# pkuyzy/ESC-GNN

Measured on AMD Instinct MI355X. Metric: graphs/sec + edges-aggregated/sec, NestedGIN_eff h=3 bs=128 @1/2/4/8 GPU, higher is better.
Workload: dtype f32; 1 GPU; count_cycle-shaped random regular graphs (n in 10/15/20/30), target=triangles, NestedGIN_eff h=3 layers=4 hidden=256, bs=128 per GPU (configs[1]); global_batch=128, parallelism=dp1 graph-sharded, rccl_ranks=1, ranks=1

## Files before the change

### esc-gnn_amd/_native.py

```python
import ctypes
import os
from ctypes import c_double, c_float, c_int, c_int64, c_void_p, POINTER

_HERE = os.path.dirname(os.path.abspath(__file__))
LIB_PATH = os.path.join(_HERE, "libescgnn_hip.so")
ABI_VERSION = 4

P, I64, I32, F32 = c_void_p, c_int64, c_int, c_float

class CollateArgs(ctypes.Structure):
    _fields_ = ([(n, c_int64) for n in ("B", "x_dim", "y_dim", "n_cols")] +
                [(n, c_void_p) for n in (
                    "graph_ids", "offsets", "node_ptr", "edge_ptr", "nnz_ptr", "y_ptr", "x_all", "y_all",
                    "esrc_all", "edst_all", "pos_enc_all", "pos_index_all", "pos_batch_all",
                    "in_ptr_all", "in_edge_all", "out_ptr_all", "out_edge_all", "row_ptr_all", "c_perm_all",
                    "c_rank_all", "col_ptr", "col_prefix",
                    "x", "y", "edge_index", "batch", "pos_enc", "pos_index", "pos_batch",
                    "in_ptr", "in_edge", "in_src", "out_ptr", "out_edge", "out_dst",
                    "row_ptr", "bag_idx", "bag_val", "col_row", "col_val", "col_col", "edge_attr_all", "edge_attr")] +
                [("ea_words", c_int64), ("x_long", c_void_p), ("graph_ptr", c_void_p)])

class BnFuse(ctypes.Structure):
    _fields_ = [("eps", c_float), ("momentum", c_float)] + [(n, c_void_p) for n in (
        "mean", "invstd", "running_mean", "running_var", "gamma", "beta", "scale", "shift")]
# ... 57 lines not shown
    "esc_plan_csr_scratch": [I64, I64],
    "esc_plan_csr": [P, I64, I64, P, P, P, P, P],
    "esc_embed_plan_scratch": [I64, I64, I64],
    "esc_embed_plan": [P, I64, I64, P, P, P, P, P, P, P, P, P, P],
    "esc_tune_set": [I32, I32],
    "esc_debug_gemm_occupancy": [I32],
    "esc_linear_bwd_input": [P, I64, P, I64, I64, I64, I64, P, I64, I32, P],
    "esc_linear_bwd_weight_scratch": [I64, I64, I64],
    "esc_linear_bwd_weight": [P, I64, P, I64, P, P, I64, I64, I64, P, I64, P, P, P],
    "esc_linear_bwd_both": [P, I64, P, I64, P, P, P, I64, I64, I64, I64, P, I64, I32, P, I64, P, P, P],
    "esc_linear_bwd_both_deferred": [P, I64, P, I64, P, P, P, I64, I64, I64, I64, P, I64, I32, P, I64, P, P, P, P],
    "esc_slab_reduce_jobs": [P, I32, P],
    "esc_linear_bwd_both_bn_ok": [P, I64, POINTER(BnBwdFused), P, I64, P, I64, I64, I64, I64, P, I64, P, POINTER(BnBwdNext)],
    "esc_linear_bwd_bn_block_rows": [I64, I64, I64],
    "esc_linear_bwd_set_wgrad_stream": [P],
    "esc_linear_bwd_both_bn": [P, I64, POINTER(BnBwdFused), P, I64, P, P, P, I64, I64, I64, I64, P, I64, I32, P, I64, P, P, P,
                               POINTER(BnBwdNext), P],
    "esc_bn_bwd_coef": [P, I64, P, I64, P, I64, I64, I64, P, P, P, P, I32, P, P, P, P, P],
    "esc_bn_bwd_coef_from_partials": [P, I64, I64, I64, P, P, P, P],
    "esc_bn_scratch": [I64],
    "esc_bn_stats": [P, I64, I64, I64, F32, F32, P, P, P, P, P, P, P, P, P, P],
    "esc_bn_stats_from_partials": [P, I64, I64, F32, F32, P, P, P, P, P, P, P, P, P],
    "esc_bn_apply": [P, I64, I64, I64, P, P, P, P, I32, P, I64, P],
    "esc_bn_bwd": [P, I64, P, I64, P, I64, I64, I64, P, P, P, P, I32, P, I64, P, P, P, P],
    "esc_bn_bwd_sums": [P, I64, P, I64, P, I64, I64, I64, P, P, P, P, I32, P, P, P, P, P],
    "esc_bn_bwd_apply": [P, I64, P, I64, P, I64, I64, I64, P, P, P, P, I32, P, P, I64, P],
    "esc_affine_act": [P, I64, I64, I64, P, P, I32, P, I64, P],
    "esc_bn_eval_coef": [P, P, P, P, F32, I64, P, P, P],
    "esc_engine_set_side_stream": [I32],
    "esc_engine_set_materialise_edge_act": [I32],
# ... 130 lines not shown
```

### esc-gnn_amd/csrc/engine.hip

```cpp
#include "common.h"

#include <cstring>
#include <map>
#include <vector>
#include <cstdlib>

namespace esc {

struct Arena {
  float* base;
  int64_t off;
  float* take(int64_t n) {
    float* p = base ? base + off : nullptr;
    off += (n + 63) & ~63LL;
    return p;
  }
};

struct BnWs { float *mean, *invstd, *scale, *shift, *nglob, *coef; };
struct MlpWs { float *Y0, *Y1; BnWs b0, b1; float* A1 = nullptr; };

struct Layout {
  int64_t N, E, Z, H, L, C0, W;
  float *Zb, *Yz; BnWs zb0, zb1;
// ... 165 lines not shown

struct SideStream {
  hipStream_t stream = nullptr;
  hipEvent_t fork_f = nullptr, join_f = nullptr, fork_b = nullptr, join_b = nullptr;
  bool ok = false;
};
static int g_materialise_edge_act = 1;
static int g_use_side_stream = 0;

struct EdgeStream {
  hipStream_t stream = nullptr;
  hipEvent_t z_ready = nullptr, joined = nullptr, lin1_fork = nullptr, lin1_rest = nullptr, tail_dz = nullptr, e_ready[ESC_MAX_LAYERS] = {}, de_ready[ESC_MAX_LAYERS] = {},
             agg_done[ESC_MAX_LAYERS] = {};
  bool ok = false;
};
static int g_split_last_lin = getenv("ESC_SPLIT_LAST_LIN") ? atoi(getenv("ESC_SPLIT_LAST_LIN")) : 1;
static int g_edge_priority_low = 1;
static int g_use_edge_stream = 1;
static int current_device() {
  int dev = 0;
  (void)hipGetDevice(&dev);
  return dev;
}
static EdgeStream& edge_stream() {
  static thread_local std::map<int, EdgeStream> per_device;
  static thread_local EdgeStream off;
  if (!g_use_edge_stream) return off;
  EdgeStream& es = per_device[current_device()];
  if (!es.ok && es.stream == nullptr) {
    int least = 0, greatest = 0;
// ... 562 lines not shown
    (void)hipEventRecord(ss.join_b, ss.stream);
  }
  Ctx ce = es.ok ? edge_ctx(c, es.stream) : c;
  std::vector<esc_reduce_job> edge_jobs;
  edge_jobs.reserve(ESC_MAX_REDUCE_JOBS);
  if (es.ok && c.jobs) ce.jobs = &edge_jobs;
  std::vector<esc_sum_job> eps_jobs;
  int64_t agg_slots = 0;
  for (int l = (int)L - 1; l >= 0; --l) {
    const esc_conv_t& cv = m->conv[l];
    const int64_t C = l == 0 ? y.C0 : H;
    const float* hin = l == 0 ? b->x : y.cat + (int64_t)l * H;
    const int64_t ld_h = l == 0 ? y.C0 : W;
    Ctx cl = c;
    if (c.wgrad) { cl.y.dT1 = y.dT1_l[l]; cl.y.dT2 = y.dT2_l[l]; }
    ESC_TRY(mlp_backward(cl, cv.nn, y.conv[l], y.agg[l], C, N, y.cat + (int64_t)(l + 1) * H, W,
                         y.dcat + (int64_t)(l + 1) * H, W, y.dagg, C, fuse_node_act(c), l == (int)L - 1 ? last_slots : agg_slots));
    agg_slots = 0;
    float* dx = l == 0 ? nullptr : y.dcat + (int64_t)l * H;
    if (split_lin1 && l == (int)L - 1 &&
        hipStreamWaitEvent((hipStream_t)c.s, es.lin1_rest, 0) != hipSuccess) { set_error("esc_engine: stream event failed"); return ESC_ELAUNCH; }
    const bool stats_here = fuse_node_act(c) && l > 0 && (g_bn_fuse_bwd & 8) && esc_gine_aggregate_bwd_deps_slots(C) == 1 && C <= 2048 &&
                            mlp_backward_fused(c, m->conv[l - 1].nn, y.conv[l - 1], y.agg[l - 1], l - 1 == 0 ? y.C0 : H, N, y.cat + (int64_t)l * H, W,
                                               y.dcat + (int64_t)l * H, W, y.dagg, l - 1 == 0 ? y.C0 : H, true);
    if (stats_here) {
      ESC_TRY(esc_gine_aggregate_bwd_affine_stats(hin, ld_h, y.cat_scale + (int64_t)l * H, y.cat_shift + (int64_t)l * H, y.conv[l - 1].b1.mean,
                                                  y.conv[l - 1].b1.invstd, y.e[l], y.ld_e[l], y.dagg, C, b->out_ptr, b->out_edge, b->out_dst, cv.eps, N, C,
                                                  y.d_e[l], C, dx, W, 1, y.deps_part + (int64_t)l * 2 * N, y.bst_part, c.s));
      agg_slots = esc_gine_aggregate_bwd_stats_slots(N);
    } else if (fuse_node_act(c) && l > 0)
      ESC_TRY(esc_gine_aggregate_bwd_affine(hin, ld_h, y.cat_scale + (int64_t)l * H, y.cat_shift + (int64_t)l * H, y.e[l], y.ld_e[l], y.dagg, C,
                                            b->out_ptr, b->out_edge, b->out_dst, cv.eps, N, C, y.d_e[l], C, dx, W, 1,
                                            y.deps_part + (int64_t)l * 2 * N, c.s));
    else
      ESC_TRY(esc_gine_aggregate_bwd(hin, ld_h, y.e[l], y.ld_e[l], y.dagg, C, b->out_ptr, b->out_edge, b->out_dst, cv.eps, N, C,
                                     y.d_e[l], C, dx, W, 1, y.deps_part + (int64_t)l * 2 * N, c.s));
    eps_jobs.push_back(esc_sum_job{y.deps_part + (int64_t)l * 2 * N, N * esc_gine_aggregate_bwd_deps_slots(C), cv.deps});
    if (es.ok) ESC_TRY(chain(es.de_ready[l], (hipStream_t)c.s, es.stream));
    const float* zin = g_materialise_edge_act ? y.Zemb : y.Yz;
    const float* zsc = g_materialise_edge_act ? nullptr : y.zb1.scale;
    const float* zsh = g_materialise_edge_act ? nullptr : y.zb1.shift;
    if (l == 0 && es.ok && c.jobs && g_split_last_lin) {
      {
        const LdsFloorGuard cap(true);
        ESC_TRY(esc_linear_bwd_input(y.d_e[l], C, cv.lin.w, H, E, C, H, y.dZemb, H, l == (int)L - 1 ? 0 : 1, es.stream));
      }
      float* slabs = *c.slab_cursor;
      *c.slab_cursor += (esc_linear_bwd_weight_scratch(E, C, H) + 63) & ~63LL;
      c.jobs->emplace_back();
      ESC_TRY(esc_linear_bwd_both_deferred(y.d_e[l], C, zin, H, zsc, zsh, cv.lin.w, H, E, C, H, nullptr, 0, 0, cv.lin.dw, H, cv.lin.db,
                                           slabs, &c.jobs->back(), c.s));
    } else {
      ESC_TRY(linear_backward(ce, y.d_e[l], C, zin, H, zsc, zsh, cv.lin, E, y.dZemb, H, l == (int)L - 1 ? 0 : 1));
// ... 952 lines not shown
```

### esc-gnn_amd/csrc/linear_mfma.hip

```cpp
#include "common.h"
#include <array>
#include <cstdlib>
#include <map>
#include "gemm_dma.h"
#include "linear_small.h"
#include <type_traits>

namespace esc {

typedef float f32x16 __attribute__((ext_vector_type(16)));

constexpr int KPAD = 4;

template <int ROWS, int BK, int NTHR = 256>
struct KContigTile {
  static constexpr int LD = BK + KPAD;
  static constexpr int FLOATS = ROWS * LD;
  static constexpr int QPR = BK / 4;
  static constexpr int PER_THREAD = ROWS * QPR / NTHR;
  static_assert(ROWS * QPR % NTHR == 0 && NTHR % QPR == 0, "tile must split evenly over the workgroup");
};
template <int COLS, int BK, int NTHR = 256>
struct RedMajorTile {
  static constexpr int LD = COLS + KPAD;
// ... 818 lines not shown
    }
  }
}

static inline bool narrow_ok(int64_t N, int64_t K, const float* X, int64_t ld_x, const float* W, int64_t ld_w,
                             const float* sc, const float* sh) {
  return N <= NARROW_N && K <= NARROW_K && K % 4 == 0 && vec_ok(X, ld_x) && vec_ok(W, ld_w) &&
         (sc == nullptr || (aligned16(sc) && aligned16(sh)));
}

enum { KNOB_FWD_BIG = 0, KNOB_FWD_SMALL = 1, KNOB_DX_BIG = 2, KNOB_DX_SMALL = 3, KNOB_DW_TILE = 4,
       KNOB_DW_BLOCKS = 5, KNOB_DW_MIN_ROWS = 6, KNOB_DUAL_SMALL = 7, KNOB_COUNT = 8 };
static int g_knob[KNOB_COUNT] = {1, 4, 1, 4, 4, 512, 128, 2};


static int g_use_dma = 15;
static inline bool dma_ok(const void* p, int64_t rows, int64_t ld) {
  return aligned16(p) && ld % 4 == 0 && rows * ld * 4 < (1LL << 31);
}
static inline bool tile128_ok(int64_t dim) { return cdiv(dim, 128) * 128 * 10 <= dim * 11; }
static inline bool dma_big(int64_t M, int64_t N) {
  if (N < 128) return false;
  if (M >= 8192) return true;
  static const int64_t min_wgs = getenv("ESC_BIG_MIN_WGS") ? atoll(getenv("ESC_BIG_MIN_WGS")) : (1LL << 62);
  return cdiv(M, 128) * cdiv(N, tile128_ok(N) ? 128 : 64) >= min_wgs;
}
static inline bool tile160_ok(int64_t dim) { return cdiv(dim, 160) * 160 * 10 <= dim * 11; }
static inline bool use160(int64_t rows, int64_t cols) {
  static const int on = getenv("ESC_TILE160") ? atoi(getenv("ESC_TILE160")) : 0;
  static const int64_t min_wgs = getenv("ESC_TILE160_MIN_WGS") ? atoll(getenv("ESC_TILE160_MIN_WGS")) : 150;
  return on && tile160_ok(cols) && cols % 128 != 0 && cdiv(rows, 128) * cdiv(cols, 160) >= min_wgs;
}
static inline hipError_t dma_check(hipError_t e, const char* what) {
  if (e != hipSuccess) set_error("%s: %s", what, hipGetErrorString(e));
  return e;
}
static void dma_wgrad_plan(int64_t M, int64_t N, int64_t K, int bm, int bn, int* splits, int* per) {
  const int64_t tiles = cdiv(N, bm) * cdiv(K, bn);
  int64_t sp = cdiv(256, tiles);
  const int64_t max_sp = cdiv(M, 128);
  if (sp > max_sp) sp = max_sp;
  if (sp < 1) sp = 1;
  int64_t pr = cdiv(cdiv(M, sp), 32) * 32;
  if (pr < 128) pr = 128;
  *per = (int)pr;
  *splits = (int)cdiv(M, pr);
}
static bool dma_fwd(const float* X, int64_t ld_x, const float* W, int64_t ld_w, const float* bias, const float* in_scale,
                    const float* in_shift, int64_t M, int64_t N, int64_t K, float* Y, int64_t ld_y, float* col_stats,
// ... 72 lines not shown
    case 3: ESC_OCC(128, 64, 2, 2, 32) break;
    case 4: ESC_OCC(64, 64, 2, 2, 64) break;
    default: ESC_OCC(64, 64, 2, 2, 32) break;
  }
#undef ESC_OCC
  return n;
}

int esc_tune_set(int knob, int value) {
  if (knob == 8) { set_last_block_finalize(value); return ESC_OK; }
  if (knob == 9) { set_norm_rowblock_cap(value); return ESC_OK; }
  if (knob == 12) { set_bn_bwd_fold(value); return ESC_OK; }
  if (knob == 13) { set_bn_bwd_one_launch(value); return ESC_OK; }
  if (knob == 10) { set_edge_lds_floor(value); return ESC_OK; }
  if (knob == 11) { g_use_dma = value; return ESC_OK; }
  ESC_REQUIRE(knob >= 0 && knob < KNOB_COUNT, "esc_tune_set: unknown knob %d", knob);
  g_knob[knob] = value;
  return ESC_OK;
}

#define ESC_TRY_(x) do { int rc__ = (x); if (rc__ != ESC_OK) return rc__; } while (0)
constexpr int64_t FUSE_FINALIZE_MAX_ROWS = 4096;

static int linear_fwd_impl(const float* X, int64_t ld_x, const float* W, int64_t ld_w, const float* bias,
                           const float* in_scale, const float* in_shift, int64_t M, int64_t N, int64_t K,
                           float* Y, int64_t ld_y, float* col_stats, const esc_bn_fuse* bn, void* stream) {
  ESC_REQUIRE(X && W && Y, "esc_linear_fwd: null pointer");
  ESC_REQUIRE(M >= 0 && N > 0 && K > 0 && ld_x >= K && ld_w >= K && ld_y >= N, "esc_linear_fwd: bad sizes M=%ld N=%ld K=%ld", (long)M, (long)N, (long)K);
  ESC_REQUIRE((in_scale == nullptr) == (in_shift == nullptr), "esc_linear_fwd: in_scale/in_shift must come together");
  ESC_REQUIRE(col_stats == nullptr || N > 32, "esc_linear_fwd: col_stats needs N > 32");
  ESC_REQUIRE(M < (1LL << 31) && N < (1LL << 31) && K < (1LL << 31), "esc_linear_fwd: dimension too large");
  ESC_REQUIRE(bn == nullptr || (col_stats && bn->mean && bn->invstd && M > 1), "esc_linear_bn_fwd: needs col_stats, mean, invstd and M > 1");
// ... 148 lines not shown
                         int64_t N, int64_t K, float* dX, int64_t ld_dx, int accumulate,
                         void* stream) {
  ESC_REQUIRE(dY && W && dX, "esc_linear_bwd_input: null pointer");
  ESC_REQUIRE(M >= 0 && N > 0 && K > 0 && ld_dy >= N && ld_w >= K && ld_dx >= K, "esc_linear_bwd_input: bad sizes");
  ESC_REQUIRE(M < (1LL << 31) && N < (1LL << 31) && K < (1LL << 31), "esc_linear_bwd_input: dimension too large");
  if (M == 0) return ESC_OK;
  hipStream_t s = (hipStream_t)stream;
  if (N <= 16 && K <= NARROW_K && K % 4 == 0 && vec_ok(W, ld_w) && vec_ok(dX, ld_dx)) {
    const unsigned blocks = (unsigned)(cdiv(M, 16) < 4096 ? cdiv(M, 16) : 4096);
    if (N <= 4) esc::launch(ESC_K_LINEAR, linear_narrow_dx<4>, dim3(blocks), dim3(256), 0, s, dY, ld_dy, W, ld_w, (int)M, (int)N, (int)K, dX, ld_dx, accumulate);
    else        esc::launch(ESC_K_LINEAR, linear_narrow_dx<16>, dim3(blocks), dim3(256), 0, s, dY, ld_dy, W, ld_w, (int)M, (int)N, (int)K, dX, ld_dx, accumulate);
    ESC_CHECK_LAUNCH("esc_linear_bwd_input.narrow");
    return ESC_OK;
  }
  if ((g_use_dma & 4) && K <= small::SMALL_MAX && N % 4 == 0 && N <= 1024 && aligned16(dY) && ld_dy % 4 == 0) {
    const size_t lds = (size_t)(32 + small::SMALL_MAX) * (N + 4) * sizeof(float);
    static size_t raised_to = 64 * 1024;
    if (dma_check(dma::raise_lds(small::smalln_dx<small::SMALL_MAX>, lds, raised_to), "esc_linear_bwd_input") != hipSuccess) return ESC_ELAUNCH;
    esc::launch(ESC_K_LINEAR, small::smalln_dx<small::SMALL_MAX>, dim3((unsigned)cdiv(M, 32)), dim3(256), lds, s, dY, ld_dy, W, ld_w,
                (int)M, (int)N, (int)K, dX, ld_dx, accumulate, BnbDev{});
    ESC_CHECK_LAUNCH("esc_linear_bwd_input.smalln");
    return ESC_OK;
  }
  if (dma_bwd_ok(dY, ld_dy, nullptr, 0, W, ld_w, M, N, K, dX, ld_dx, nullptr, true, false)) {
    dma::GArgs d{};
    dma_fill_dx(d, dY, ld_dy, W, ld_w, M, N, K, dX, ld_dx, accumulate);
    const hipError_t e = use160(M, K) ? dma::launch_gemm<128, 160, 32, 4, 1, 3, 4, false, true, 0, false, false>(d, 0, s)
                         : (M >= 8192 && tile128_ok(K)) ? dma::launch_gemm<128, 128, 32, 2, 2, 3, 4, false, true, 0, false, false>(d, 0, s)
                                   : dma::launch_gemm<64, 64, 32, 2, 2, 3, 2, false, true, 0, false, false>(d, 0, s);
    return dma_check(e, "esc_linear_bwd_input") == hipSuccess ? ESC_OK : ESC_ELAUNCH;
  }
  GemmArgs g{};
  g.A = dY; g.lda = ld_dy; g.B = W; g.ldb = ld_w; g.C = dX; g.ldc = ld_dx; g.bias = nullptr;
  g.rowsC = (int)M; g.colsC = (int)K; g.red = (int)N; g.red_per_split = (int)N; g.accumulate = accumulate;
  g.a_vec = vec_ok(dY, ld_dy); g.b_vec = vec_ok(W, ld_w); g.c_slab = 0;
// ... 49 lines not shown

static int weight_impl(const float* dY, int64_t ld_dy, const float* X, int64_t ld_x, const float* in_scale,
                       const float* in_shift, int64_t M, int64_t N, int64_t K, float* dW, int64_t ld_dw, float* db,
                       float* slabs, esc_reduce_job* defer, void* stream) {
  ESC_REQUIRE(dY && X && dW && slabs, "esc_linear_bwd_weight: null pointer");
  ESC_REQUIRE(M > 0 && N > 0 && K > 0 && ld_dy >= N && ld_x >= K && ld_dw >= K, "esc_linear_bwd_weight: bad sizes");
  ESC_REQUIRE((in_scale == nullptr) == (in_shift == nullptr), "esc_linear_bwd_weight: in_scale/in_shift must come together");
  ESC_REQUIRE(M < (1LL << 31) && N < (1LL << 31) && K < (1LL << 31), "esc_linear_bwd_weight: dimension too large");
  hipStream_t s = (hipStream_t)stream;
  int splits, per;
  if ((g_use_dma & 4) && (K <= small::SMALL_MAX) != (N <= small::SMALL_MAX)) {
    splits = (int)cdiv(M, small::ROWS_WGRAD);
    float* db_part = slabs + (size_t)splits * N * K;
    const bool small_k = K <= small::SMALL_MAX;
    const dim3 grid((unsigned)splits, (unsigned)cdiv(small_k ? N : K, 256));
#define ESC_WGRAD_SMALL(SK, PR) esc::launch(ESC_K_LINEAR, small::wgrad_small<small::SMALL_MAX, SK, PR>, grid, dim3(256), 0, s, dY, ld_dy, X, ld_x, in_scale, in_shift, (int)M, (int)N, (int)K, slabs, db_part, BnbDev{})
    if (small_k) { if (in_scale) ESC_WGRAD_SMALL(true, true); else ESC_WGRAD_SMALL(true, false); }
    else         { if (in_scale) ESC_WGRAD_SMALL(false, true); else ESC_WGRAD_SMALL(false, false); }
#undef ESC_WGRAD_SMALL
    ESC_CHECK_LAUNCH("esc_linear_bwd_weight.small");
    const int64_t n = N * K;
    if (defer) { fill_job(defer, slabs, n, splits, K, dW, ld_dw, db_part, N, db); return ESC_OK; }
    esc::launch(ESC_K_LINEAR, slab_reduce_kernel, dim3((unsigned)cdiv(n + (db ? N : 0), 256)), dim3(256), 0, s, slabs, n,
                splits, (int)K, dW, ld_dw, db_part, (int)N, db);
    ESC_CHECK_LAUNCH("esc_linear_bwd_weight.reduce");
    return ESC_OK;
  }
  if (dma_bwd_ok(dY, ld_dy, X, ld_x, nullptr, 0, M, N, K, nullptr, 0, slabs, false, true)) {
    const bool big = M >= 8192 && tile128_ok(N) && tile128_ok(K);
    dma_wgrad_plan(M, N, K, big ? 128 : 64, big ? 128 : 64, &splits, &per);
    dma::GArgs d{};
    dma_fill_dw(d, dY, ld_dy, X, ld_x, in_scale, in_shift, M, N, K, slabs, splits, per);
    hipError_t e;
// ... 157 lines not shown
    else if (big) e = in_scale ? dma::launch_dual<128, 128, 32, 2, 2, 3, 4, true>(a, 0, s)
                          : dma::launch_dual<128, 128, 32, 2, 2, 3, 4, false>(a, 0, s);
    else {
      hipStream_t sw = defer ? wgrad_stream_after(s) : s;
      e = in_scale ? dma::launch_dual<64, 64, 32, 2, 2, 3, 2, true>(a, 0, s, ESC_K_LINEAR, sw) : dma::launch_dual<64, 64, 32, 2, 2, 3, 2, false>(a, 0, s, ESC_K_LINEAR, sw);
    }
    if (dma_check(e, "esc_linear_bwd_both") != hipSuccess) return ESC_ELAUNCH;
    const int64_t n = N * K;
    if (defer) { fill_job(defer, slabs, n, splits, K, dW, ld_dw, a.dw.db_part, N, db); return ESC_OK; }
    esc::launch(ESC_K_LINEAR, slab_reduce_kernel, dim3((unsigned)cdiv(n + (db ? N : 0), 256)), dim3(256), 0, s, slabs, n,
                splits, (int)K, dW, ld_dw, a.dw.db_part, (int)N, db);
    ESC_CHECK_LAUNCH("esc_linear_bwd_both.reduce");
    return ESC_OK;
  }
  if (dX == nullptr || N <= 32 || K <= 32) {
    int rc = weight_impl(dY, ld_dy, X, ld_x, in_scale, in_shift, M, N, K, dW, ld_dw, db, slabs, defer, stream);
    if (rc || dX == nullptr) return rc;
    return esc_linear_bwd_input(dY, ld_dy, W, ld_w, M, N, K, dX, ld_dx, accumulate, stream);
  }
  ESC_REQUIRE(M > 0 && ld_dy >= N && ld_x >= K && ld_w >= K && ld_dx >= K && ld_dw >= K, "esc_linear_bwd_both: bad sizes");
  ESC_REQUIRE((in_scale == nullptr) == (in_shift == nullptr), "esc_linear_bwd_both: in_scale/in_shift must come together");
  ESC_REQUIRE(M < (1LL << 31) && N < (1LL << 31) && K < (1LL << 31), "esc_linear_bwd_both: dimension too large");
  hipStream_t s = (hipStream_t)stream;
  const int small_tile = g_knob[KNOB_DUAL_SMALL];
  const int bm = (M >= 8192 || small_tile != 1) ? 64 : 32, bn = 64;
  const int bk = (M >= 8192 || small_tile != 0) ? 32 : 64;
  int splits, per;
  wgrad_plan_tile(M, N, K, bm, bn, bk, &splits, &per);
  DualArgs a{};
  GemmArgs& g = a.dx;
  g.A = dY; g.lda = ld_dy; g.B = W; g.ldb = ld_w; g.C = dX; g.ldc = ld_dx;
  g.rowsC = (int)M; g.colsC = (int)K; g.red = (int)N; g.red_per_split = (int)N; g.accumulate = accumulate;
// ... 20 lines not shown
}


static inline BnbDev bnb_dev(const esc_bn_bwd_fused* b) {
  return BnbDev{b->x, (int)b->ld_x, b->mean, b->invstd, b->scale, b->shift, reinterpret_cast<const float2*>(b->coef), b->relu};
}
static inline bool bnb_operands_ok(const esc_bn_bwd_fused* b, int64_t M, int64_t N) {
  return b && b->x && b->mean && b->invstd && b->scale && b->shift && b->coef && b->relu >= 0 && b->relu <= 2 && b->ld_x >= N &&
         dma_ok(b->x, M, b->ld_x) && aligned16(b->mean) && aligned16(b->invstd) && aligned16(b->scale) && aligned16(b->shift) &&
         aligned16(b->coef);
}
static inline bool bnb_big_shape(int64_t M, int64_t N, int64_t K) { return M >= 8192 && tile128_ok(N) && tile128_ok(K); }
static inline bool in_range_big(int64_t N) { return N <= 640; }
static inline bool bnb_small_shape(int64_t N, int64_t K) { return (g_use_dma & 4) && K <= small::SMALL_MAX && N > small::SMALL_MAX && N % 4 == 0 && N <= 1024; }

int esc_linear_bwd_set_wgrad_stream(void* stream) {
  g_wside.stream = (hipStream_t)stream;
  return ESC_OK;
}

int esc_linear_bwd_both_bn_ok(const float* dOut, int64_t ld_dout, const esc_bn_bwd_fused* bn, const float* X, int64_t ld_x,
                              const float* W, int64_t ld_w, int64_t M, int64_t N, int64_t K, const float* dX, int64_t ld_dx,
                              const float* slabs, const esc_bn_bwd_next* next) {
  if (!dOut || !X || !W || !slabs || M <= 1 || N <= 0 || K <= 0 || (bn == nullptr && next == nullptr)) return 0;
  if (M >= 8192 && !(bnb_big_shape(M, N, K) && bn != nullptr && in_range_big(N))) return 0;
  if (bn != nullptr && !bnb_operands_ok(bn, M, N)) return 0;
  if (bn != nullptr && bnb_small_shape(N, K))
    return next == nullptr && aligned16(dOut) && ld_dout % 4 == 0 && ld_dout >= N && ld_x >= K && ld_w >= K && (dX == nullptr || ld_dx >= K);
  if (dX == nullptr || N > dma::Cfg<64, 64, 32, 2, 2, 2, 2, false, true, 4, false, false>::BNB_MAXK) return 0;
  if (!dma_bwd_ok(dOut, ld_dout, X, ld_x, W, ld_w, M, N, K, dX, ld_dx, slabs, true, true)) return 0;
// ... 11 lines not shown
int esc_linear_bwd_both_bn(const float* dOut, int64_t ld_dout, const esc_bn_bwd_fused* bn, const float* X, int64_t ld_x,
                           const float* in_scale, const float* in_shift, const float* W, int64_t ld_w, int64_t M,
                           int64_t N, int64_t K, float* dX, int64_t ld_dx, int accumulate, float* dW, int64_t ld_dw,
                           float* db, float* slabs, esc_reduce_job* defer, const esc_bn_bwd_next* next, void* stream) {
  ESC_REQUIRE(dOut && X && W && dW && slabs, "esc_linear_bwd_both_bn: null pointer");
  ESC_REQUIRE((in_scale == nullptr) == (in_shift == nullptr), "esc_linear_bwd_both_bn: in_scale/in_shift must come together");
  ESC_REQUIRE(ld_dw >= K, "esc_linear_bwd_both_bn: bad sizes");
  ESC_REQUIRE(esc_linear_bwd_both_bn_ok(dOut, ld_dout, bn, X, ld_x, W, ld_w, M, N, K, dX, ld_dx, slabs, next),
              "esc_linear_bwd_both_bn: shape / alignment not served (M=%ld N=%ld K=%ld) - use esc_bn_bwd + esc_linear_bwd_both", (long)M, (long)N, (long)K);
  hipStream_t s = (hipStream_t)stream;
  const BnbDev bd = bn ? bnb_dev(bn) : BnbDev{};
  const int64_t n = N * K;
  if (bn && bnb_small_shape(N, K)) {
    const int splits = (int)cdiv(M, small::ROWS_WGRAD);
    float* db_part = slabs + (size_t)splits * N * K;
    const dim3 grid((unsigned)splits, (unsigned)cdiv(N, 256));
    hipStream_t sw = defer ? wgrad_stream_after(s) : s;
#define ESC_WG(PR, ACT) esc::launch(ESC_K_LINEAR, small::wgrad_small<small::SMALL_MAX, true, PR, ACT>, grid, dim3(256), 0, sw, dOut, ld_dout, X, ld_x, in_scale, in_shift, (int)M, (int)N, (int)K, slabs, db_part, bd)
    if (bd.relu == 2) { if (in_scale) ESC_WG(true, 2); else ESC_WG(false, 2); }
    else              { if (in_scale) ESC_WG(true, 1); else ESC_WG(false, 1); }
#undef ESC_WG
    ESC_CHECK_LAUNCH("esc_linear_bwd_both_bn.small");
    if (dX != nullptr) {
      const size_t lds = (size_t)(32 + small::SMALL_MAX) * (N + 4) * sizeof(float);
      static size_t raised_to = 64 * 1024;
      auto kern = bd.relu == 2 ? small::smalln_dx<small::SMALL_MAX, 2> : small::smalln_dx<small::SMALL_MAX, 1>;
      if (dma_check(dma::raise_lds(small::smalln_dx<small::SMALL_MAX, 1>, lds, raised_to), "esc_linear_bwd_both_bn") != hipSuccess) return ESC_ELAUNCH;
      static size_t raised_elu = 64 * 1024;
      if (bd.relu == 2 && dma_check(dma::raise_lds(small::smalln_dx<small::SMALL_MAX, 2>, lds, raised_elu), "esc_linear_bwd_both_bn") != hipSuccess) return ESC_ELAUNCH;
      esc::launch(ESC_K_LINEAR, kern, dim3((unsigned)cdiv(M, 32)), dim3(256), lds, s, dOut, ld_dout, W, ld_w, (int)M, (int)N, (int)K, dX, ld_dx, accumulate, bd);
      ESC_CHECK_LAUNCH("esc_linear_bwd_both_bn.smalln");
    }
    if (defer) { fill_job(defer, slabs, n, splits, K, dW, ld_dw, db_part, N, db); return ESC_OK; }
    esc::launch(ESC_K_LINEAR, slab_reduce_kernel, dim3((unsigned)cdiv(n + (db ? N : 0), 256)), dim3(256), 0, s, slabs, n,
                splits, (int)K, dW, ld_dw, db_part, (int)N, db);
    ESC_CHECK_LAUNCH("esc_linear_bwd_both_bn.reduce");
    return ESC_OK;
  }
  const bool big = bnb_big_shape(M, N, K);
  int splits, per;
  dma_wgrad_plan(M, N, K, big ? 128 : 64, big ? 128 : 64, &splits, &per);
  dma::DualArgs a{};
  dma_fill_dx(a.dx, dOut, ld_dout, W, ld_w, M, N, K, dX, ld_dx, accumulate);
  dma_fill_dw(a.dw, dOut, ld_dout, X, ld_x, in_scale, in_shift, M, N, K, slabs, splits, per);
  a.dx.bnb = bd; a.dw.bnb = bd;
  if (next)
    a.dx.bst = BnStatDev{reinterpret_cast<float2*>(next->partial), next->x, (int)next->ld_x, next->mean, next->invstd, next->scale, next->shift, next->relu};
// ... 21 lines not shown
```

### esc-gnn_amd/csrc/linear_small.h

```cpp
#pragma once
#include "common.h"

namespace esc {
namespace small {

constexpr int SMALL_MAX = 16;
constexpr int ROWS_FWD = 32;
constexpr int ROWS_WGRAD = 32;

template <int KMAX>
__global__ __launch_bounds__(256) void smallk_fwd(const float* __restrict__ X, int64_t ldx, const float* __restrict__ W,
                                                  int64_t ldw, const float* __restrict__ bias, int M, int N, int K,
                                                  float* __restrict__ Y, int64_t ldy, float2* __restrict__ col_stats) {
  ESC_PRIO();
  __shared__ float xs[ROWS_FWD * KMAX];
  const int n = blockIdx.y * 256 + threadIdx.x;
  const int r0 = blockIdx.x * ROWS_FWD;
  const int rows = min(ROWS_FWD, M - r0);
  for (int i = threadIdx.x; i < ROWS_FWD * KMAX; i += 256) {
    const int r = i / KMAX, k = i % KMAX;
    xs[i] = (r < rows && k < K) ? X[(size_t)(r0 + r) * ldx + k] : 0.f;
  }
  float w[KMAX];
#pragma unroll
// ... 125 lines not shown
    const int k = ks + kk * 8;
    if (k >= K) break;
    float a0 = 0.f, a1 = 0.f, a2 = 0.f, a3 = 0.f;
    for (int c = 0; c < N; c += 4) {
      const float4 y = *reinterpret_cast<const float4*>(ys + r * ldn + c);
      const float4 w = *reinterpret_cast<const float4*>(wt + k * ldn + c);
      a0 = fmaf(y.x, w.x, a0); a1 = fmaf(y.y, w.y, a1); a2 = fmaf(y.z, w.z, a2); a3 = fmaf(y.w, w.w, a3);
    }
    float v = (a0 + a1) + (a2 + a3);
    float* dst = dX + (size_t)(r0 + r) * lddx + k;
    if (accumulate) v += *dst;
    *dst = v;
  }
}

}
}
```

### include/escgnn_hip.h

```cpp
#ifndef ESCGNN_HIP_H
#define ESCGNN_HIP_H

#include <stdint.h>

#ifdef __cplusplus
extern "C" {
#endif

#define ESC_OK 0
#define ESC_EINVAL (-1)
#define ESC_ELAUNCH (-2)
#define ESC_ERANGE (-3)

int esc_abi_version(void);
const char* esc_last_error(void);

enum { ESC_K_AGG_FWD = 0, ESC_K_AGG_BWD = 1, ESC_K_BAG_FWD = 2, ESC_K_BAG_BWD = 3,
       ESC_K_LINEAR = 4, ESC_K_COLLATE = 5, ESC_K_FEATURES = 6, ESC_K_NORM = 7,
       ESC_K_GEMM_EDGE = 8,
       ESC_K_COUNT = 9 };
int esc_prof_enable(int kind, int on);
int esc_prof_read(int kind, int64_t* launches, double* total_ms);
int64_t esc_prof_read_all(int kind, double* ms_out, int64_t cap);
int esc_prof_reset(int kind);
// ... 138 lines not shown
  const float* coef;
  int32_t relu;
} esc_bn_bwd_fused;
typedef struct esc_bn_bwd_next {
  float* partial;
  const float* x; int64_t ld_x;
  const float* mean; const float* invstd; const float* scale; const float* shift;
  int32_t relu;
} esc_bn_bwd_next;
int esc_linear_bwd_both_bn_ok(const float* dOut, int64_t ld_dout, const esc_bn_bwd_fused* bn, const float* X, int64_t ld_x,
                              const float* W, int64_t ld_w, int64_t M, int64_t N, int64_t K, const float* dX, int64_t ld_dx,
                              const float* slabs, const esc_bn_bwd_next* next);
int64_t esc_linear_bwd_bn_block_rows(int64_t M, int64_t N, int64_t K);

int esc_linear_bwd_set_wgrad_stream(void* stream);
int esc_linear_bwd_both_bn(const float* dOut, int64_t ld_dout, const esc_bn_bwd_fused* bn, const float* X, int64_t ld_x,
                           const float* in_scale, const float* in_shift, const float* W, int64_t ld_w, int64_t M,
                           int64_t N, int64_t K, float* dX, int64_t ld_dx, int accumulate, float* dW, int64_t ld_dw,
                           float* db, float* slabs, esc_reduce_job* job, const esc_bn_bwd_next* next, void* stream);
int esc_bn_bwd_coef(const float* X, int64_t ld_x, const float* Y, int64_t ld_y, const float* dY, int64_t ld_dy, int64_t M,
                    int64_t C, const float* mean, const float* invstd, const float* gamma, const float* beta, int relu,
                    float* coef, float* dgamma, float* dbeta, float* scratch, void* stream);
int esc_bn_bwd_coef_from_partials(const float* partial, int64_t slots, int64_t M, int64_t C, float* coef, float* dgamma,
                                  float* dbeta, void* stream);

int64_t esc_bn_scratch(int64_t C);
int esc_bn_stats(const float* X, int64_t ld_x, int64_t M, int64_t C, float eps, float momentum,
                 float* mean, float* invstd, float* running_mean, float* running_var,
                 const float* gamma, const float* beta, float* scale, float* shift,
                 float* scratch, void* stream);
// ... 219 lines not shown
```

Before: 130,000 graphs/s.

## Add v2 small-K linear backward kernels and defer layer-0 weight-grad launch

Adds new register-tiled small-K weight-gradient and dX kernels (v2) that use static LDS and are enabled by default through a new knob. The layer-0 small weight-gradient launch can now be held and released after the edge-stream handoff, so the dX critical path runs first. The small-shape path also issues dX before wgrad by default. The v2 kernels change the thread mapping and LDS usage, which may shift occupancy, and the reordering changes stream overlap behaviour.

```diff
diff --git a/esc-gnn_amd/_native.py b/esc-gnn_amd/_native.py
--- a/esc-gnn_amd/_native.py
+++ b/esc-gnn_amd/_native.py
@@ -95,6 +95,8 @@
     "esc_linear_bwd_both_bn_ok": [P, I64, POINTER(BnBwdFused), P, I64, P, I64, I64, I64, I64, P, I64, P, POINTER(BnBwdNext)],
     "esc_linear_bwd_bn_block_rows": [I64, I64, I64],
     "esc_linear_bwd_set_wgrad_stream": [P],
+    "esc_linear_bwd_hold_wgrad": [I32],
+    "esc_linear_bwd_release_wgrad": [P],
     "esc_linear_bwd_both_bn": [P, I64, POINTER(BnBwdFused), P, I64, P, P, P, I64, I64, I64, I64, P, I64, I32, P, I64, P, P, P,
                                POINTER(BnBwdNext), P],
     "esc_bn_bwd_coef": [P, I64, P, I64, P, I64, I64, I64, P, P, P, P, I32, P, P, P, P, P],
diff --git a/esc-gnn_amd/csrc/engine.hip b/esc-gnn_amd/csrc/engine.hip
--- a/esc-gnn_amd/csrc/engine.hip
+++ b/esc-gnn_amd/csrc/engine.hip
@@ -203,6 +203,7 @@
              agg_done[ESC_MAX_LAYERS] = {};
   bool ok = false;
 };
+static int g_defer_wgrad0 = getenv("ESC_DEFER_WGRAD0") ? atoi(getenv("ESC_DEFER_WGRAD0")) : 1;
 static int g_split_last_lin = getenv("ESC_SPLIT_LAST_LIN") ? atoi(getenv("ESC_SPLIT_LAST_LIN")) : 1;
 static int g_edge_priority_low = 1;
 static int g_use_edge_stream = 1;
@@ -795,8 +796,12 @@
     const int64_t ld_h = l == 0 ? y.C0 : W;
     Ctx cl = c;
     if (c.wgrad) { cl.y.dT1 = y.dT1_l[l]; cl.y.dT2 = y.dT2_l[l]; }
-    ESC_TRY(mlp_backward(cl, cv.nn, y.conv[l], y.agg[l], C, N, y.cat + (int64_t)(l + 1) * H, W,
-                         y.dcat + (int64_t)(l + 1) * H, W, y.dagg, C, fuse_node_act(c), l == (int)L - 1 ? last_slots : agg_slots));
+    const bool hold0 = l == 0 && g_defer_wgrad0 && es.ok && c.jobs != nullptr && c.wgrad == nullptr;
+    if (hold0) (void)esc_linear_bwd_hold_wgrad(1);
+    const int rc_mlp = mlp_backward(cl, cv.nn, y.conv[l], y.agg[l], C, N, y.cat + (int64_t)(l + 1) * H, W,
+                                    y.dcat + (int64_t)(l + 1) * H, W, y.dagg, C, fuse_node_act(c), l == (int)L - 1 ? last_slots : agg_slots);
+    if (hold0) (void)esc_linear_bwd_hold_wgrad(0);
+    ESC_TRY(rc_mlp);
     agg_slots = 0;
     float* dx = l == 0 ? nullptr : y.dcat + (int64_t)l * H;
     if (split_lin1 && l == (int)L - 1 &&
@@ -818,6 +823,7 @@
                                      y.d_e[l], C, dx, W, 1, y.deps_part + (int64_t)l * 2 * N, c.s));
     eps_jobs.push_back(esc_sum_job{y.deps_part + (int64_t)l * 2 * N, N * esc_gine_aggregate_bwd_deps_slots(C), cv.deps});
     if (es.ok) ESC_TRY(chain(es.de_ready[l], (hipStream_t)c.s, es.stream));
+    if (hold0) ESC_TRY(esc_linear_bwd_release_wgrad(c.s));
     const float* zin = g_materialise_edge_act ? y.Zemb : y.Yz;
     const float* zsc = g_materialise_edge_act ? nullptr : y.zb1.scale;
     const float* zsh = g_materialise_edge_act ? nullptr : y.zb1.shift;
diff --git a/esc-gnn_amd/csrc/linear_mfma.hip b/esc-gnn_amd/csrc/linear_mfma.hip
--- a/esc-gnn_amd/csrc/linear_mfma.hip
+++ b/esc-gnn_amd/csrc/linear_mfma.hip
@@ -856,6 +856,7 @@
 static int g_knob[KNOB_COUNT] = {1, 4, 1, 4, 4, 512, 128, 2};
 
 
+static int g_small_gen = getenv("ESC_SMALL_LINEAR") ? atoi(getenv("ESC_SMALL_LINEAR")) : 7;
 static int g_use_dma = 15;
 static inline bool dma_ok(const void* p, int64_t rows, int64_t ld) {
   return aligned16(p) && ld % 4 == 0 && rows * ld * 4 < (1LL << 31);
@@ -874,7 +875,10 @@
   return on && tile160_ok(cols) && cols % 128 != 0 && cdiv(rows, 128) * cdiv(cols, 160) >= min_wgs;
 }
 static inline hipError_t dma_check(hipError_t e, const char* what) {
-  if (e != hipSuccess) set_error("%s: %s", what, hipGetErrorString(e));
+  if (e != hipSuccess) {
+    set_error("%s: %s", what, hipGetErrorString(e));
+    (void)hipGetLastError();
+  }
   return e;
 }
 static void dma_wgrad_plan(int64_t M, int64_t N, int64_t K, int bm, int bn, int* splits, int* per) {
@@ -977,8 +981,26 @@
   if (knob == 13) { set_bn_bwd_one_launch(value); return ESC_OK; }
   if (knob == 10) { set_edge_lds_floor(value); return ESC_OK; }
   if (knob == 11) { g_use_dma = value; return ESC_OK; }
+  if (knob == 14) { g_small_gen = value; return ESC_OK; }
   ESC_REQUIRE(knob >= 0 && knob < KNOB_COUNT, "esc_tune_set: unknown knob %d", knob);
   g_knob[knob] = value;
+  return ESC_OK;
+}
+
+static int launch_smalln_dx(const float* dY, int64_t ld_dy, const float* W, int64_t ld_w, int64_t M, int64_t N, int64_t K, float* dX,
+                            int64_t ld_dx, int accumulate, const BnbDev& bd, int bnb_mode, hipStream_t s, const char* who) {
+  constexpr int SM = small::SMALL_MAX;
+  if (g_small_gen & 1) {
+    const dim3 grid((unsigned)cdiv(M, small::DX2_ROWS));
+    auto kern = bnb_mode == 2 ? small::smalln_dx_v2<SM, 2> : bnb_mode == 1 ? small::smalln_dx_v2<SM, 1> : small::smalln_dx_v2<SM, 0>;
+    esc::launch(ESC_K_LINEAR, kern, grid, dim3(256), 0, s, dY, ld_dy, W, ld_w, (int)M, (int)N, (int)K, dX, ld_dx, accumulate, bd);
+    return ESC_OK;
+  }
+  const size_t lds = (size_t)(32 + SM) * (N + 4) * sizeof(float);
+  static size_t raised[3] = {64 * 1024, 64 * 1024, 64 * 1024};
+  auto kern = bnb_mode == 2 ? small::smalln_dx<SM, 2> : bnb_mode == 1 ? small::smalln_dx<SM, 1> : small::smalln_dx<SM, 0>;
+  if (dma_check(dma::raise_lds(kern, lds, raised[bnb_mode]), who) != hipSuccess) return ESC_ELAUNCH;
+  esc::launch(ESC_K_LINEAR, kern, dim3((unsigned)cdiv(M, 32)), dim3(256), lds, s, dY, ld_dy, W, ld_w, (int)M, (int)N, (int)K, dX, ld_dx, accumulate, bd);
   return ESC_OK;
 }
 
@@ -1157,11 +1179,7 @@
     return ESC_OK;
   }
   if ((g_use_dma & 4) && K <= small::SMALL_MAX && N % 4 == 0 && N <= 1024 && aligned16(dY) && ld_dy % 4 == 0) {
-    const size_t lds = (size_t)(32 + small::SMALL_MAX) * (N + 4) * sizeof(float);
-    static size_t raised_to = 64 * 1024;
-    if (dma_check(dma::raise_lds(small::smalln_dx<small::SMALL_MAX>, lds, raised_to), "esc_linear_bwd_input") != hipSuccess) return ESC_ELAUNCH;
-    esc::launch(ESC_K_LINEAR, small::smalln_dx<small::SMALL_MAX>, dim3((unsigned)cdiv(M, 32)), dim3(256), lds, s, dY, ld_dy, W, ld_w,
-                (int)M, (int)N, (int)K, dX, ld_dx, accumulate, BnbDev{});
+    if (int rc = launch_smalln_dx(dY, ld_dy, W, ld_w, M, N, K, dX, ld_dx, accumulate, BnbDev{}, 0, s, "esc_linear_bwd_input")) return rc;
     ESC_CHECK_LAUNCH("esc_linear_bwd_input.smalln");
     return ESC_OK;
   }
@@ -1241,9 +1259,11 @@
     float* db_part = slabs + (size_t)splits * N * K;
     const bool small_k = K <= small::SMALL_MAX;
     const dim3 grid((unsigned)splits, (unsigned)cdiv(small_k ? N : K, 256));
-#define ESC_WGRAD_SMALL(SK, PR) esc::launch(ESC_K_LINEAR, small::wgrad_small<small::SMALL_MAX, SK, PR>, grid, dim3(256), 0, s, dY, ld_dy, X, ld_x, in_scale, in_shift, (int)M, (int)N, (int)K, slabs, db_part, BnbDev{})
-    if (small_k) { if (in_scale) ESC_WGRAD_SMALL(true, true); else ESC_WGRAD_SMALL(true, false); }
-    else         { if (in_scale) ESC_WGRAD_SMALL(false, true); else ESC_WGRAD_SMALL(false, false); }
+#define ESC_WGRAD_SMALL(SK, PR) \
+    if (g_small_gen & 1) esc::launch(ESC_K_LINEAR, small::wgrad_small_v2<small::SMALL_MAX, SK, PR>, grid, dim3(256), 0, s, dY, ld_dy, X, ld_x, in_scale, in_shift, (int)M, (int)N, (int)K, slabs, db_part, BnbDev{}); \
+    else                 esc::launch(ESC_K_LINEAR, small::wgrad_small<small::SMALL_MAX, SK, PR>, grid, dim3(256), 0, s, dY, ld_dy, X, ld_x, in_scale, in_shift, (int)M, (int)N, (int)K, slabs, db_part, BnbDev{})
+    if (small_k) { if (in_scale) { ESC_WGRAD_SMALL(true, true); } else { ESC_WGRAD_SMALL(true, false); } }
+    else         { if (in_scale) { ESC_WGRAD_SMALL(false, true); } else { ESC_WGRAD_SMALL(false, false); } }
 #undef ESC_WGRAD_SMALL
     ESC_CHECK_LAUNCH("esc_linear_bwd_weight.small");
     const int64_t n = N * K;
@@ -1431,8 +1451,9 @@
     return ESC_OK;
   }
   if (dX == nullptr || N <= 32 || K <= 32) {
+    if (dX != nullptr && (g_small_gen & 2)) ESC_TRY_(esc_linear_bwd_input(dY, ld_dy, W, ld_w, M, N, K, dX, ld_dx, accumulate, stream));
     int rc = weight_impl(dY, ld_dy, X, ld_x, in_scale, in_shift, M, N, K, dW, ld_dw, db, slabs, defer, stream);
-    if (rc || dX == nullptr) return rc;
+    if (rc || dX == nullptr || (g_small_gen & 2)) return rc;
     return esc_linear_bwd_input(dY, ld_dy, W, ld_w, M, N, K, dX, ld_dx, accumulate, stream);
   }
   ESC_REQUIRE(M > 0 && ld_dy >= N && ld_x >= K && ld_w >= K && ld_dx >= K && ld_dw >= K, "esc_linear_bwd_both: bad sizes");
@@ -1483,6 +1504,37 @@
 static inline bool in_range_big(int64_t N) { return N <= 640; }
 static inline bool bnb_small_shape(int64_t N, int64_t K) { return (g_use_dma & 4) && K <= small::SMALL_MAX && N > small::SMALL_MAX && N % 4 == 0 && N <= 1024; }
 
+struct SmallWgrad {
+  const float* dOut; int64_t ld_dout; const float* X; int64_t ld_x; const float* in_scale; const float* in_shift;
+  int M, N, K; float* slabs; float* db_part; BnbDev bd;
+};
+static void launch_small_wgrad(const SmallWgrad& w, hipStream_t s) {
+  const dim3 grid((unsigned)cdiv(w.M, small::ROWS_WGRAD), (unsigned)cdiv(w.N, 256));
+#define ESC_WG(PR, ACT) \
+  if (g_small_gen & 1) esc::launch(ESC_K_LINEAR, small::wgrad_small_v2<small::SMALL_MAX, true, PR, ACT>, grid, dim3(256), 0, s, w.dOut, w.ld_dout, w.X, w.ld_x, w.in_scale, w.in_shift, w.M, w.N, w.K, w.slabs, w.db_part, w.bd); \
+  else                 esc::launch(ESC_K_LINEAR, small::wgrad_small<small::SMALL_MAX, true, PR, ACT>, grid, dim3(256), 0, s, w.dOut, w.ld_dout, w.X, w.ld_x, w.in_scale, w.in_shift, w.M, w.N, w.K, w.slabs, w.db_part, w.bd)
+  if (w.bd.relu == 2) { if (w.in_scale) { ESC_WG(true, 2); } else { ESC_WG(false, 2); } }
+  else                { if (w.in_scale) { ESC_WG(true, 1); } else { ESC_WG(false, 1); } }
+#undef ESC_WG
+}
+struct HeldWgrad { bool armed = false, have = false; SmallWgrad job{}; };
+static thread_local HeldWgrad g_held;
+
+int esc_linear_bwd_hold_wgrad(int on) {
+  g_held.armed = on != 0;
+  if (on) g_held.have = false;
+  return ESC_OK;
+}
+
+int esc_linear_bwd_release_wgrad(void* stream) {
+  g_held.armed = false;
+  if (!g_held.have) return ESC_OK;
+  g_held.have = false;
+  launch_small_wgrad(g_held.job, (hipStream_t)stream);
+  ESC_CHECK_LAUNCH("esc_linear_bwd_release_wgrad");
+  return ESC_OK;
+}
+
 int esc_linear_bwd_set_wgrad_stream(void* stream) {
   g_wside.stream = (hipStream_t)stream;
   return ESC_OK;
@@ -1524,23 +1576,17 @@
   if (bn && bnb_small_shape(N, K)) {
     const int splits = (int)cdiv(M, small::ROWS_WGRAD);
     float* db_part = slabs + (size_t)splits * N * K;
-    const dim3 grid((unsigned)splits, (unsigned)cdiv(N, 256));
+    const SmallWgrad wg{dOut, ld_dout, X, ld_x, in_scale, in_shift, (int)M, (int)N, (int)K, slabs, db_part, bd};
     hipStream_t sw = defer ? wgrad_stream_after(s) : s;
-#define ESC_WG(PR, ACT) esc::launch(ESC_K_LINEAR, small::wgrad_small<small::SMALL_MAX, true, PR, ACT>, grid, dim3(256), 0, sw, dOut, ld_dout, X, ld_x, in_scale, in_shift, (int)M, (int)N, (int)K, slabs, db_part, bd)
-    if (bd.relu == 2) { if (in_scale) ESC_WG(true, 2); else ESC_WG(false, 2); }
-    else              { if (in_scale) ESC_WG(true, 1); else ESC_WG(false, 1); }
-#undef ESC_WG
-    ESC_CHECK_LAUNCH("esc_linear_bwd_both_bn.small");
+    const bool hold = (g_small_gen & 4) && g_held.armed && defer != nullptr && dX != nullptr && sw == s;
+    const bool dx_first = hold || (g_small_gen & 2);
+    if (!dx_first) { launch_small_wgrad(wg, sw); ESC_CHECK_LAUNCH("esc_linear_bwd_both_bn.small"); }
     if (dX != nullptr) {
-      const size_t lds = (size_t)(32 + small::SMALL_MAX) * (N + 4) * sizeof(float);
-      static size_t raised_to = 64 * 1024;
-      auto kern = bd.relu == 2 ? small::smalln_dx<small::SMALL_MAX, 2> : small::smalln_dx<small::SMALL_MAX, 1>;
-      if (dma_check(dma::raise_lds(small::smalln_dx<small::SMALL_MAX, 1>, lds, raised_to), "esc_linear_bwd_both_bn") != hipSuccess) return ESC_ELAUNCH;
-      static size_t raised_elu = 64 * 1024;
-      if (bd.relu == 2 && dma_check(dma::raise_lds(small::smalln_dx<small::SMALL_MAX, 2>, lds, raised_elu), "esc_linear_bwd_both_bn") != hipSuccess) return ESC_ELAUNCH;
-      esc::launch(ESC_K_LINEAR, kern, dim3((unsigned)cdiv(M, 32)), dim3(256), lds, s, dOut, ld_dout, W, ld_w, (int)M, (int)N, (int)K, dX, ld_dx, accumulate, bd);
+      if (int rc = launch_smalln_dx(dOut, ld_dout, W, ld_w, M, N, K, dX, ld_dx, accumulate, bd, bd.relu == 2 ? 2 : 1, s, "esc_linear_bwd_both_bn")) return rc;
       ESC_CHECK_LAUNCH("esc_linear_bwd_both_bn.smalln");
     }
+    if (hold) { g_held.job = wg; g_held.have = true; }
+    else if (dx_first) { launch_small_wgrad(wg, sw); ESC_CHECK_LAUNCH("esc_linear_bwd_both_bn.small"); }
     if (defer) { fill_job(defer, slabs, n, splits, K, dW, ld_dw, db_part, N, db); return ESC_OK; }
     esc::launch(ESC_K_LINEAR, slab_reduce_kernel, dim3((unsigned)cdiv(n + (db ? N : 0), 256)), dim3(256), 0, s, slabs, n,
                 splits, (int)K, dW, ld_dw, db_part, (int)N, db);
diff --git a/esc-gnn_amd/csrc/linear_small.h b/esc-gnn_amd/csrc/linear_small.h
--- a/esc-gnn_amd/csrc/linear_small.h
+++ b/esc-gnn_amd/csrc/linear_small.h
@@ -163,5 +163,180 @@
   }
 }
 
-}
-}
+
+
+template <int SMAX, bool SMALL_K, bool PRO, int BNB = 0>
+__global__ __launch_bounds__(256) void wgrad_small_v2(const float* __restrict__ dY, int64_t lddy, const float* __restrict__ X,
+                                                      int64_t ldx, const float* __restrict__ sc, const float* __restrict__ sh,
+                                                      int M, int N, int K, float* __restrict__ slabs, float* __restrict__ db_part,
+                                                      BnbDev bnb) {
+  static_assert(BNB == 0 || SMALL_K, "the fused BatchNorm backward transforms the wide dY operand");
+  static_assert((ROWS_WGRAD * SMAX) % 256 == 0, "whole passes over the uniform tile");
+  ESC_PRIO();
+  __shared__ __attribute__((aligned(16))) float us[ROWS_WGRAD * SMAX];
+  const int t = blockIdx.y * 256 + threadIdx.x;
+  const int split = blockIdx.x;
+  const int r0 = split * ROWS_WGRAD;
+  const int rows = min(ROWS_WGRAD, M - r0);
+  const int S = SMALL_K ? K : N;
+  const int Wd = SMALL_K ? N : K;
+  const float* U = SMALL_K ? X : dY;
+  const int64_t ldu = SMALL_K ? ldx : lddy;
+  const float* V = SMALL_K ? dY : X;
+  const int64_t ldv = SMALL_K ? lddy : ldx;
+  const bool live = t < Wd;
+  constexpr int UPT = ROWS_WGRAD * SMAX / 256;
+  float u[UPT], usc[UPT], ush[UPT];
+#pragma unroll
+  for (int j = 0; j < UPT; ++j) {
+    const int i = threadIdx.x + j * 256, r = i / SMAX, q = i % SMAX;
+    const bool in = r < rows && q < S;
+    u[j] = in ? U[(size_t)(r0 + r) * ldu + q] : 0.f;
+    if constexpr (PRO && SMALL_K) { usc[j] = in ? sc[q] : 0.f; ush[j] = in ? sh[q] : 0.f; }
+  }
+  float v[ROWS_WGRAD], xb[ROWS_WGRAD];
+  const int tc = min(t, Wd - 1);
+#pragma unroll
+  for (int r = 0; r < ROWS_WGRAD; ++r) {
+    const int rc = r0 + min(r, rows - 1);
+    v[r] = V[(size_t)rc * ldv + tc];
+    if constexpr (BNB != 0) xb[r] = bnb.x[(size_t)rc * bnb.ldx + tc];
+  }
+  float psc = 1.f, psh = 0.f;
+  if constexpr (PRO && !SMALL_K) { if (live) { psc = sc[t]; psh = sh[t]; } }
+  float b_mu = 0.f, b_a = 0.f, b_ms = 0.f, b_mh = 1.f, b_k1 = 0.f, b_k2 = 0.f;
+  if constexpr (BNB != 0) {
+    if (live) {
+      const float2 kk = bnb.coef[t];
+      b_mu = bnb.mean[t]; b_a = bnb.scale[t]; b_k1 = kk.x; b_k2 = bnb.invstd[t] * kk.y;
+      if (bnb.relu) { b_ms = b_a; b_mh = bnb.shift[t]; }
+    }
+  }
+#pragma unroll
+  for (int j = 0; j < UPT; ++j) {
+    const int i = threadIdx.x + j * 256, r = i / SMAX, q = i % SMAX;
+    float w = u[j];
+    if constexpr (PRO && SMALL_K) { if (r < rows && q < S) w = fmaxf(fmaf(w, usc[j], ush[j]), 0.f); }
+    us[i] = w;
+  }
+  __syncthreads();
+  float acc[SMAX];
+#pragma unroll
+  for (int q = 0; q < SMAX; ++q) acc[q] = 0.f;
+  float colsum = 0.f;
+  if (live) {
+#pragma unroll
+    for (int r = 0; r < ROWS_WGRAD; ++r) {
+      if (r < rows) {
+        float w = v[r];
+        if constexpr (BNB == 1) w = bnb_apply(w, xb[r], b_mu, b_a, b_ms, b_mh, b_k1, b_k2);
+        if constexpr (BNB == 2) w = bnb_apply_elu(w, xb[r], b_mu, b_a, b_ms, b_mh, b_k1, b_k2);
+        if constexpr (PRO && !SMALL_K) w = fmaxf(fmaf(w, psc, psh), 0.f);
+        if constexpr (SMALL_K) colsum += w;
+#pragma unroll
+        for (int q = 0; q < SMAX; ++q) acc[q] = fmaf(us[r * SMAX + q], w, acc[q]);
+      }
+    }
+    float* out = slabs + (size_t)split * N * K;
+#pragma unroll
+    for (int q = 0; q < SMAX; ++q)
+      if (q < S) out[SMALL_K ? (size_t)t * K + q : (size_t)q * K + t] = acc[q];
+    if constexpr (SMALL_K) db_part[(size_t)split * N + t] = colsum;
+  }
+  if constexpr (!SMALL_K) {
+    if (blockIdx.y == 0 && (int)threadIdx.x < N) {
+      float s = 0.f;
+      for (int r = 0; r < rows; ++r) s += us[r * SMAX + threadIdx.x];
+      db_part[(size_t)split * N + threadIdx.x] = s;
+    }
+  }
+}
+
+constexpr int DX2_ROWS = 16;
+constexpr int DX2_NC = 256;
+constexpr int DX2_LD = DX2_NC + 4;
+constexpr int DX2_LDS_FLOATS = (DX2_ROWS + 16) * DX2_LD;
+template <int KMAX, int BNB = 0>
+__global__ __launch_bounds__(256) void smalln_dx_v2(const float* __restrict__ dY, int64_t lddy, const float* __restrict__ W,
+                                                    int64_t ldw, int M, int N, int K, float* __restrict__ dX, int64_t lddx,
+                                                    int accumulate, BnbDev bnb) {
+  static_assert(KMAX == 16, "thread map: 16 rows x 16 k-slots");
+  ESC_PRIO();
+  __shared__ __attribute__((aligned(16))) float sm[DX2_LDS_FLOATS];
+  float* ys = sm;
+  float* wt = sm + DX2_ROWS * DX2_LD;
+  const int r0 = blockIdx.x * DX2_ROWS;
+  const int rows = min(DX2_ROWS, M - r0);
+  const int cg = threadIdx.x & 63, rl = threadIdx.x >> 6;
+  const int r = threadIdx.x >> 4, k = threadIdx.x & 15;
+  const bool out = r < rows && k < K;
+  float a0 = 0.f, a1 = 0.f, a2 = 0.f, a3 = 0.f;
+  for (int n0 = 0; n0 < N; n0 += DX2_NC) {
+    const int nc = min(DX2_NC, N - n0);
+    const int c = cg * 4;
+    const bool colin = c < nc;
+    float4 g[DX2_ROWS / 4], x[DX2_ROWS / 4];
+#pragma unroll
+    for (int j = 0; j < DX2_ROWS / 4; ++j) {
+      const int rr = rl + 4 * j;
+      const bool in = colin && rr < rows;
+      g[j] = in ? *reinterpret_cast<const float4*>(dY + (size_t)(r0 + rr) * lddy + n0 + c) : make_float4(0.f, 0.f, 0.f, 0.f);
+      if constexpr (BNB != 0)
+        x[j] = in ? *reinterpret_cast<const float4*>(bnb.x + (size_t)(r0 + rr) * bnb.ldx + n0 + c) : make_float4(0.f, 0.f, 0.f, 0.f);
+    }
+    float4 mu{}, a{}, is{}, k01{}, k23{}, ms = make_float4(0.f, 0.f, 0.f, 0.f), mh = make_float4(1.f, 1.f, 1.f, 1.f);
+    if constexpr (BNB != 0) {
+      if (colin) {
+        mu = *reinterpret_cast<const float4*>(bnb.mean + n0 + c); a = *reinterpret_cast<const float4*>(bnb.scale + n0 + c);
+        is = *reinterpret_cast<const float4*>(bnb.invstd + n0 + c);
+        k01 = *reinterpret_cast<const float4*>(bnb.coef + n0 + c); k23 = *reinterpret_cast<const float4*>(bnb.coef + n0 + c + 2);
+        if (bnb.relu) { ms = a; mh = *reinterpret_cast<const float4*>(bnb.shift + n0 + c); }
+      }
+    }
+    float wr[KMAX];
+    const bool win = (int)threadIdx.x < nc;
+#pragma unroll
+    for (int q = 0; q < KMAX; ++q) wr[q] = (win && q < K) ? W[(size_t)(n0 + threadIdx.x) * ldw + q] : 0.f;
+    if (n0 > 0) __syncthreads();
+#pragma unroll
+    for (int j = 0; j < DX2_ROWS / 4; ++j) {
+      const int rr = rl + 4 * j;
+      float4 v = g[j];
+      if constexpr (BNB != 0) {
+        if (colin && rr < rows) {
+          const float4 xx = x[j];
+          if constexpr (BNB == 2) {
+            v.x = bnb_apply_elu(v.x, xx.x, mu.x, a.x, ms.x, mh.x, k01.x, is.x * k01.y); v.y = bnb_apply_elu(v.y, xx.y, mu.y, a.y, ms.y, mh.y, k01.z, is.y * k01.w);
+            v.z = bnb_apply_elu(v.z, xx.z, mu.z, a.z, ms.z, mh.z, k23.x, is.z * k23.y); v.w = bnb_apply_elu(v.w, xx.w, mu.w, a.w, ms.w, mh.w, k23.z, is.w * k23.w);
+          } else {
+            v.x = bnb_apply(v.x, xx.x, mu.x, a.x, ms.x, mh.x, k01.x, is.x * k01.y); v.y = bnb_apply(v.y, xx.y, mu.y, a.y, ms.y, mh.y, k01.z, is.y * k01.w);
+            v.z = bnb_apply(v.z, xx.z, mu.z, a.z, ms.z, mh.z, k23.x, is.z * k23.y); v.w = bnb_apply(v.w, xx.w, mu.w, a.w, ms.w, mh.w, k23.z, is.w * k23.w);
+          }
+        }
+      }
+      if (colin && rr < rows) *reinterpret_cast<float4*>(ys + rr * DX2_LD + c) = v;
+    }
+    if (win) {
+#pragma unroll
+      for (int q = 0; q < KMAX; ++q) wt[q * DX2_LD + threadIdx.x] = wr[q];
+    }
+    __syncthreads();
+    if (out) {
+#pragma unroll 4
+      for (int cc = 0; cc < nc; cc += 4) {
+        const float4 y = *reinterpret_cast<const float4*>(ys + r * DX2_LD + cc);
+        const float4 w = *reinterpret_cast<const float4*>(wt + k * DX2_LD + cc);
+        a0 = fmaf(y.x, w.x, a0); a1 = fmaf(y.y, w.y, a1); a2 = fmaf(y.z, w.z, a2); a3 = fmaf(y.w, w.w, a3);
+      }
+    }
+  }
+  if (out) {
+    float v = (a0 + a1) + (a2 + a3);
+    float* dst = dX + (size_t)(r0 + r) * lddx + k;
+    if (accumulate) v += *dst;
+    *dst = v;
+  }
+}
+
+}
+}
diff --git a/include/escgnn_hip.h b/include/escgnn_hip.h
--- a/include/escgnn_hip.h
+++ b/include/escgnn_hip.h
@@ -176,6 +176,8 @@
 int64_t esc_linear_bwd_bn_block_rows(int64_t M, int64_t N, int64_t K);
 
 int esc_linear_bwd_set_wgrad_stream(void* stream);
+int esc_linear_bwd_hold_wgrad(int on);
+int esc_linear_bwd_release_wgrad(void* stream);
 int esc_linear_bwd_both_bn(const float* dOut, int64_t ld_dout, const esc_bn_bwd_fused* bn, const float* X, int64_t ld_x,
                            const float* in_scale, const float* in_shift, const float* W, int64_t ld_w, int64_t M,
                            int64_t N, int64_t K, float* dX, int64_t ld_dx, int accumulate, float* dW, int64_t ld_dw,
```

New measurement: 130,900 graphs/s, median of 6. Within noise of the previous version (+0.7%).
